# HanielUlises/GCN-GrabCut

Hardware: AMD Instinct MI355X
Metric: images/sec end-to-end mask (DUTS-shape batch) (higher is better)
Workload: dtype f32

## Files before the change

### gcn-grabcut_amd/csrc/ggc_gc.h

```cpp
#pragma once
#include "ggc_internal.h"

namespace ggc {

constexpr int DINF = 1 << 29;

struct GcDims { int B, H, W, P, n_chunks; };

__device__ __forceinline__ int dir_dx(int dir) { return (dir == 0 || dir == 4 || dir == 7) ? -1 : ((dir == 1 || dir == 5 || dir == 6) ? 1 : 0); }
__device__ __forceinline__ int dir_dy(int dir) { return (dir == 2 || dir == 4 || dir == 6) ? -1 : ((dir == 3 || dir == 5 || dir == 7) ? 1 : 0); }
__device__ __forceinline__ int dir_nb(const GcDims& d, int y, int x, int dir) {
    const int yy = y + dir_dy(dir), xx = x + dir_dx(dir);
    if (xx < 0 || xx >= d.W || yy < 0 || yy >= d.H) return -1;
    return yy * d.W + xx;
}

__host__ __device__ __forceinline__ size_t rc_idx(int dir, size_t i) { return i * 8 + (size_t)dir; }

__device__ __forceinline__ void mf_cold_pixel(size_t i, int32_t tw, const int32_t (&cap)[8], int32_t* __restrict__ rc,
                                              int32_t* __restrict__ ex, int32_t* __restrict__ snk, uint8_t* __restrict__ rmask) {
    int arcs = 0;
    int4* r = reinterpret_cast<int4*>(rc + rc_idx(0, i));
    r[0] = make_int4(cap[0], cap[1], cap[2], cap[3]);
    r[1] = make_int4(cap[4], cap[5], cap[6], cap[7]);
#pragma unroll
    for (int dir = 0; dir < 8; ++dir) arcs |= cap[dir] > 0 ? 1 << dir : 0;
    rmask[i] = (uint8_t)arcs;
    ex[i] = tw > 0 ? tw : 0;
    snk[i] = tw < 0 ? -tw : 0;
}

__device__ __forceinline__ void mf_plane_caps(const GcDims& d, int b, int p, const int32_t* __restrict__ nw, int32_t (&cap)[8]) {
    const size_t BP = (size_t)d.B * d.P;
    const int y = p / d.W, x = p % d.W;
    const int32_t* nwb = nw + (size_t)b * d.P;
    const int dirs[4] = {0, 4, 2, 6};
#pragma unroll
    for (int k = 0; k < 4; ++k) {
        const int dir = dirs[k];
        cap[dir] = dir_nb(d, y, x, dir) >= 0 ? nwb[(size_t)k * BP + p] : 0;
        const int q = dir_nb(d, y, x, dir ^ 1);
        cap[dir ^ 1] = q >= 0 ? nwb[(size_t)k * BP + q] : 0;
    }
}

__device__ __forceinline__ void mf_warm_pixel(size_t i, int32_t tw, int32_t tw_old, int32_t* __restrict__ ex,
                                              int32_t* __restrict__ snk) {
    const int32_t bal = (ex[i] - snk[i]) + (tw - tw_old);
    ex[i] = bal > 0 ? bal : 0;
    snk[i] = bal < 0 ? -bal : 0;
}

struct MfControl {
    int32_t* active;
    int32_t* cnt;
    int32_t* lists;
    int32_t* err;
};

int maxflow(ggc_ctx* ctx, hipStream_t st, const GcDims& d, const int32_t* state, int32_t* rc, int32_t* ex,
            int32_t* snk, int32_t* dist, uint8_t* rmask, const MfControl& ctl, bool masks_exact, int& n_open);

constexpr int MF_RT = 32;
constexpr int MF_PT_W = 32, MF_PT_H = 8;
struct MfTiles { int rt_x, rt_y, pt_x, pt_y; };

void mf_zero3(hipStream_t st, int32_t* a, size_t na, int32_t* b, size_t nb, int32_t* c, size_t nc);

constexpr int AQ_HEAD = 0, AQ_TAIL = 32, AQ_PENDING = 64, AQ_DONE = 96, AQ_BUDGET = 97, AQ_VISITS = 128, AQ_WORDS = 160;
int maxflow_relax_async(ggc_ctx* ctx, hipStream_t st, const GcDims& d, const MfTiles& tl, uint8_t* rmask, int32_t* dirty, const int32_t* rc, int32_t* dist,
                        const int32_t* count, const int32_t* list, int32_t* flag, unsigned long long* ring, int32_t* q, int cap,
                        int grid, int32_t* err_flag);
int maxflow_push_async(ggc_ctx* ctx, hipStream_t st, const GcDims& d, const MfTiles& tl, int th, int inner, int gen_max, int32_t* rc,
                       int32_t* ex, int32_t* snk, int32_t* dist, uint8_t* rmask, int32_t* dirty, const int32_t* count, const int32_t* list, int n_list_max, int32_t* state,
                       unsigned long long* ring, int32_t* q, int waves, int32_t* err_flag, long long* prof = nullptr);

}
```

### gcn-grabcut_amd/csrc/ggc_maxflow.hip

```cpp
#include "ggc_gc.h"
#include "ggc_mf_sweep.h"
#include <algorithm>
#include <chrono>
#include <cstdlib>
#include <vector>

namespace ggc {

constexpr int RT = MF_RT;
constexpr int PT_W = MF_PT_W, PT_H = MF_PT_H;
constexpr int PT_N = PT_W * PT_H;
constexpr int PUSH_GRID = 1024, RELAX_GRID = 1024, ASYNC_GRID = 128;

__global__ void __launch_bounds__(256) k_mf_zero3(int32_t* __restrict__ a, size_t na, int32_t* __restrict__ b, size_t nb, int32_t* __restrict__ c, size_t nc) {
    const size_t i = (size_t)blockIdx.x * 256 + threadIdx.x;
    if (i < na) a[i] = 0;
    else if (i < na + nb) b[i - na] = 0;
    else if (i < na + nb + nc) c[i - na - nb] = 0;
}
void mf_zero3(hipStream_t st, int32_t* a, size_t na, int32_t* b, size_t nb, int32_t* c, size_t nc) {
    const size_t n = na + nb + nc;
    if (n) hipLaunchKernelGGL(k_mf_zero3, dim3(cdiv(n, 256)), dim3(256), 0, st, a, na, b, nb, c, nc);
}

// ... 1 lines not shown
struct OutList { int n, base; int buf[OUT_CAP]; };
__device__ __forceinline__ void push_tile_l(int tile, int32_t* __restrict__ flag, OutList& L, int32_t* __restrict__ list,
                                            int32_t* __restrict__ count) {
    if (ldg(&flag[tile]) == 0 && atomicExch(&flag[tile], 1) == 0) {
        const int i = atomicAdd(&L.n, 1);
        if (i < OUT_CAP) L.buf[i] = tile;
        else list[atomicAdd(count, 1)] = tile;
    }
}
__device__ __forceinline__ void flush_tiles(OutList& L, int32_t* __restrict__ list, int32_t* __restrict__ count) {
    __syncthreads();
    const int n = min(L.n, OUT_CAP);
    if (threadIdx.x == 0 && n > 0) L.base = atomicAdd(count, n);
    __syncthreads();
    for (int i = threadIdx.x; i < n; i += blockDim.x) list[L.base + i] = L.buf[i];
}

__global__ void __launch_bounds__(256) k_mf_rinit(GcDims d, MfTiles tl, const int32_t* __restrict__ open_list,
                                                  const int32_t* __restrict__ snk, int32_t* __restrict__ dist,
                                                  int32_t* __restrict__ list, int32_t* __restrict__ flag, int32_t* __restrict__ flag2,
                                                  int32_t* __restrict__ count, int32_t* __restrict__ active, int32_t* __restrict__ scan) {
    constexpr int T = MF_RT;
    __shared__ OutList outl;
    if (threadIdx.x == 0) outl.n = 0;
    if (blockIdx.x == 0 && threadIdx.x == 0) active[open_list[blockIdx.y]] = 0;
    if (blockIdx.x == 0 && blockIdx.y == 0 && threadIdx.x < 8 && (threadIdx.x == 0 || threadIdx.x >= 4)) scan[threadIdx.x] = 0;
    __syncthreads();
    const int tiles_per_image = tl.rt_x * tl.rt_y;
    const int tr = blockIdx.x * 4 + (threadIdx.x >> 6), lane = threadIdx.x & 63;
    if (tr < tiles_per_image) {
        const int b = open_list[blockIdx.y];
        const int ty0 = (tr / tl.rt_x) * T, tx0 = (tr % tl.rt_x) * T;
        const int lx = lane & 31, h = lane >> 5;
        const size_t base = (size_t)b * d.P;
        int sv[16];
#pragma unroll
        for (int r = 0; r < 16; ++r) sv[r] = snk[base + (size_t)min(ty0 + 16 * h + r, d.H - 1) * d.W + min(tx0 + lx, d.W - 1)];
        bool open_px = false;
#pragma unroll
        for (int r = 0; r < 16; ++r) {
            const int y = ty0 + 16 * h + r, x = tx0 + lx;
            if (x < d.W && y < d.H) {
                dist[base + (size_t)y * d.W + x] = sv[r] > 0 ? 1 : DINF;
                open_px |= sv[r] <= 0;
            }
        }
        const bool listed = __any(open_px);
        if (lane == 0) {
            const int tile = b * tiles_per_image + tr;
            flag[tile] = listed ? 1 : 0;
            flag2[tile] = 0;
            if (listed) {
                const int i = atomicAdd(&outl.n, 1);
                if (i < OUT_CAP) outl.buf[i] = tile; else list[atomicAdd(count, 1)] = tile;
            }
        }
    }
    flush_tiles(outl, list, count);
}

template <bool PROF>
__global__ void __launch_bounds__(256) k_mf_relax_wave(GcDims d, MfTiles tl, int phase, long long* __restrict__ prof, uint8_t* __restrict__ rmask,
                                                       int32_t* __restrict__ dirty, const int32_t* __restrict__ rc, int32_t* __restrict__ dist, int32_t* __restrict__ counters,
                                                       const int32_t* __restrict__ list_in, int32_t* __restrict__ list_out,
                                                       int32_t* __restrict__ flag_in, int32_t* __restrict__ flag_out) {
    __shared__ RelaxWaveLds lds[4];
    __shared__ OutList outl;
    if (threadIdx.x == 0) outl.n = 0;
    __syncthreads();
    const int wv = threadIdx.x >> 6;
    const int n_in = counters[phase % 3];
    int32_t* n_out = counters + (phase + 1) % 3;
    if (blockIdx.x == 0 && threadIdx.x == 0) counters[(phase + 2) % 3] = 0;
    const int tiles_per_image = tl.rt_x * tl.rt_y;
    const int G = gridDim.x * 4;
    MfRelaxClocks<PROF> ck;
    int tile_nx = blockIdx.x * 4 + wv < n_in ? list_in[blockIdx.x * 4 + wv] : 0;
    for (int t = blockIdx.x * 4 + wv; t < n_in; t += G) {
        int lane = threadIdx.x & 63;
        asm volatile("" : "+v"(lane));
        ck.begin();
        const int tile = __builtin_amdgcn_readfirstlane(tile_nx);
        tile_nx = t + G < n_in ? list_in[t + G] : 0;
        const int nbm = mf_relax_visit<false, PROF, GGC_MF_RELAX_BFS != 0>(d, tl, tile, lane, lds[wv], rmask, dirty, rc, dist, flag_in, ck);
        const int b = tile / tiles_per_image, tr = tile % tiles_per_image;
        const int tyi = tr / tl.rt_x, txi = tr % tl.rt_x;
        if (lane < 9 && (nbm >> lane) & 1) {
            const int ty = tyi + lane / 3 - 1, tx = txi + lane % 3 - 1;
            if (ty >= 0 && ty < tl.rt_y && tx >= 0 && tx < tl.rt_x)
                push_tile_l(b * tiles_per_image + ty * tl.rt_x + tx, flag_out, outl, list_out, n_out);
        }
        mf_wave_sync();
        ck.end();
    }
    if (PROF && (threadIdx.x & 63) == 0 && ck.sum[3]) {
        unsigned long long* q = reinterpret_cast<unsigned long long*>(prof) + (64 + (blockIdx.x & 63)) * 8;
        for (int k = 0; k < 7; ++k) atomicAdd(&q[k], (unsigned long long)ck.sum[k]);
    }
    flush_tiles(outl, list_out, n_out);
}

__global__ void __launch_bounds__(PT_N) k_mf_pr_list(GcDims d, MfTiles tl, int phase, int inner,
                                                    int32_t* __restrict__ rc, int32_t* __restrict__ ex,
                                                    int32_t* __restrict__ snk, int32_t* __restrict__ dist, uint8_t* __restrict__ rmask,
                                                    int32_t* __restrict__ dirty, int32_t* __restrict__ counters, const int32_t* __restrict__ list_in,
                                                    int32_t* __restrict__ list_out, int32_t* __restrict__ flag_in,
                                                    int32_t* __restrict__ flag_out) {
    __shared__ int s_ex[PT_N];
    __shared__ int s_d[PT_H + 2][PT_W + 2];
    __shared__ int s_rc[8][PT_N];
    __shared__ OutList outl;
    __shared__ int s_nbm;
    const int tid = threadIdx.x, lx = tid & 31;
    if (tid == 0) outl.n = 0;
    const int n_in = counters[phase % 3];
    int32_t* n_out = counters + (phase + 1) % 3;
    if (blockIdx.x == 0 && tid == 0) counters[(phase + 2) % 3] = 0;
    const int tiles_per_image = tl.pt_x * tl.pt_y;
    const size_t BP = (size_t)d.B * d.P;
    constexpr int N_HALO = (PT_H + 2) * (PT_W + 2), HALO_IT = (N_HALO + PT_N - 1) / PT_N;
    struct TileRegs { int e, sk, r[8], hv[HALO_IT]; };
    auto load_tile = [&](int tile, TileRegs& R) {
        const int b = tile / tiles_per_image, tr = tile % tiles_per_image;
        const int tyi = tr / tl.pt_x, txi = tr % tl.pt_x;
        const int x = txi * PT_W + lx;
        const size_t base = (size_t)b * d.P;
        const int y = tyi * PT_H + (tid >> 5);
        const bool in = x < d.W && y < d.H;
        const int p = y * d.W + x;
        R.e = in ? ex[base + p] : 0;
        R.sk = in ? snk[base + p] : 0;
#pragma unroll
        for (int dir = 0; dir < 8; ++dir) R.r[dir] = in ? rc[rc_idx(dir, base + p)] : 0;
#pragma unroll
        for (int k = 0; k < HALO_IT; ++k) {
            const int i = tid + k * PT_N;
            const int gy = tyi * PT_H + i / (PT_W + 2) - 1, gx = txi * PT_W + i % (PT_W + 2) - 1;
            R.hv[k] = (i < N_HALO && gx >= 0 && gx < d.W && gy >= 0 && gy < d.H) ? dist[base + (size_t)gy * d.W + gx] : DINF;
        }
    };
    const int G = gridDim.x;
    int t = blockIdx.x;
    if (t >= n_in) return;
    int tile_next = list_in[t];
    int tile_next2 = t + G < n_in ? list_in[t + G] : 0;
    TileRegs N;
    load_tile(tile_next, N);
    for (; t < n_in; t += G) {
        const int tile = tile_next;
        const int b = tile / tiles_per_image, tr = tile % tiles_per_image;
        const int tyi = tr / tl.pt_x, txi = tr % tl.pt_x;
        const int x = txi * PT_W + lx;
        const size_t base = (size_t)b * d.P;
        __syncthreads();
        const int y = tyi * PT_H + (tid >> 5);
        const bool inb = x < d.W && y < d.H;
        const int pp = y * d.W + x;
        const int e0 = N.e, sk0 = N.sk;
        int sk = sk0, r0[8];
        s_ex[tid] = e0;
#pragma unroll
        for (int dir = 0; dir < 8; ++dir) { r0[dir] = N.r[dir]; s_rc[dir][tid] = r0[dir]; }
#pragma unroll
        for (int k = 0; k < HALO_IT; ++k) {
            const int i = tid + k * PT_N;
            if (i < N_HALO) s_d[i / (PT_W + 2)][i % (PT_W + 2)] = N.hv[k];
        }
        if (t + G < n_in) {
            tile_next = tile_next2;
// ... 203 lines not shown
        launches = phase;
        if (partial) return GGC_OK;
        const int pool = (int)std::min<size_t>(ASYNC_GRID * scale, std::max<size_t>(16, cdiv((size_t)n_cur * per_image, 16)));
        launches = phase + 1;
        return maxflow_relax_async(ctx, st, d, tl, rmask, w.dirty, rc, dist, rl_cnt + phase % 3, w.rl_list[phase & 1], w.rl_flag[phase & 1],
                                   w.ring, w.aq, (int)n_rt, pool, ctl.err);
    }

    int push(int round, int n_cur, size_t scale, int total_active, int& waves) {
        const Knobs& kn = knobs();
        ProfScope ps(ctx, st, "maxflow_push");
        if (round > 0 && total_active <= kn.mf_async_push_active) {
            waves = (int)std::min<long long>(4ll * ASYNC_GRID * (long long)scale, std::max<long long>(64, total_active / 4));
            return maxflow_push_async(ctx, st, d, tl, kn.mf_async_tile, kn.mf_async_sweeps, kn.mf_async_hops, rc, ex, snk, dist, rmask, w.dirty,
                                      pr_cnt, w.pt_list[0], (int)n_pt, w.busy, w.ring, w.aq, waves, ctl.err, prof);
        }
        waves = 0;
        const int launches = round == 0 ? kn.mf_dense_launches0 : kn.mf_dense_launches;
        const int pr_grid = (int)std::min<size_t>(PUSH_GRID * scale, std::max<size_t>(64, (size_t)n_cur * tl.pt_x * tl.pt_y / 2));
        const int grid = (int)std::min<long long>(pr_grid, std::max<long long>(128, 2ll * total_active));
        for (int phase = 0; phase < launches; ++phase)
            hipLaunchKernelGGL(k_mf_pr_list, dim3(grid), dim3(PT_N), 0, st, d, tl, phase, kn.mf_dense_sweeps, rc, ex, snk, dist, rmask, w.dirty, pr_cnt,
                               w.pt_list[phase & 1], w.pt_list[(phase + 1) & 1], w.pt_flag[phase & 1], w.pt_flag[(phase + 1) & 1]);
        GGC_LAUNCH_CHECK(ctx);
        return GGC_OK;
    }
};

struct MfTrace {
    std::chrono::steady_clock::time_point t_prev = std::chrono::steady_clock::now();
    double push_ms = 0.0;

    int round(const MfSolve& s, int round, int n_next, int total_active, int relax_launches) {
        ggc_ctx* ctx = s.ctx;
        long long hh[64 * 8], h[7] = {0, 0, 0, 0, 0, 0, 0};
        GGC_HIP(ctx, hipStreamSynchronize(s.st));
        GGC_HIP(ctx, hipMemcpy(hh, s.prof + 64 * 8, sizeof hh, hipMemcpyDeviceToHost));
        GGC_HIP(ctx, hipMemsetAsync(s.prof + 64 * 8, 0, sizeof hh, s.st));
        for (int i = 0; i < 64; ++i) for (int k = 0; k < 7; ++k) h[k] += hh[i * 8 + k];
        if (h[3] > 0)
            std::fprintf(stderr, "    [relabel visits] %lld dense visits: per visit load+fill %.2f us, sweeps %.2f us (%.1f sweeps, %.1f BFS levels, %lld visits fell back), write-back %.2f us\n",
                         h[3], 0.01 * h[0] / h[3], 0.01 * h[1] / h[3], (double)h[4] / h[3], (double)h[5] / h[3], h[6], 0.01 * h[2] / h[3]);
        std::vector<int32_t> act;
        if (int rcode = read_i32(ctx, s.st, s.ctl.active, s.d.B, act)) return rcode;
        const auto t_now = std::chrono::steady_clock::now();
        const double ms = std::chrono::duration<double, std::milli>(t_now - t_prev).count();
        std::fprintf(stderr, "[ggc maxflow] round %d: open images %d, active pixels %d, relabel launches %d, relabel+scan %.3f ms, previous push %.3f ms\n",
                     round, n_next, total_active, relax_launches, ms - push_ms, push_ms);
        t_prev = t_now;
        if (n_next > 0 && n_next <= 12) {
            std::fprintf(stderr, "    [open]");
            for (int b = 0; b < s.d.B; ++b) if (act[b]) std::fprintf(stderr, " %d:%d", b, act[b]);
            std::fprintf(stderr, "\n");
        }
        return GGC_OK;
    }

    int push(const MfSolve& s, int waves) {
        ggc_ctx* ctx = s.ctx;
        GGC_HIP(ctx, hipStreamSynchronize(s.st));
        push_ms = std::chrono::duration<double, std::milli>(std::chrono::steady_clock::now() - t_prev).count();
        if (waves == 0) return GGC_OK;
        long long hh[128 * 8], h[7] = {0, 0, 0, 0, 0, 0, 0}, g[3] = {0, 0, 0};
        GGC_HIP(ctx, hipMemcpy(hh, s.prof, sizeof hh, hipMemcpyDeviceToHost));
        GGC_HIP(ctx, hipMemsetAsync(s.prof, 0, sizeof hh, s.st));
        for (int i = 0; i < 64; ++i) for (int k = 0; k < 7; ++k) h[k] += hh[i * 8 + k];
        for (int i = 0; i < 64; ++i) for (int k = 0; k < 3; ++k) g[k] += hh[(64 + i) * 8 + k];
        if (h[3] > 0)
            std::fprintf(stderr, "    [async visit] load+fill %.2f us, sweeps %.2f us (%.1f sweeps), write-back+drain %.2f us\n", 0.01 * g[0] / h[3],
                         0.01 * g[1] / h[3], (double)g[2] / h[3], 0.01 * (h[1] - g[0] - g[1]) / h[3]);
        if (h[6] > 0)
            std::fprintf(stderr, "    [async push] %d waves alive %.1f us on average; %lld visits (%lld followed): per visit wait+lock %.2f us, "
                         "visit %.2f us, hand-over %.2f us\n", waves, 0.01 * h[5] / h[6], h[3], h[4], h[3] ? 0.01 * h[0] / h[3] : 0.0,
                         h[3] ? 0.01 * h[1] / h[3] : 0.0, h[3] ? 0.01 * h[2] / h[3] : 0.0);
        return GGC_OK;
    }
};

}

int maxflow(ggc_ctx* ctx, hipStream_t st, const GcDims& d, const int32_t* state, int32_t* rc, int32_t* ex,
            int32_t* snk, int32_t* dist, uint8_t* rmask, const MfControl& ctl, bool masks_exact, int& n_open) {
    const Knobs& kn = knobs();
    const MfTiles tl{cdiv(d.W, RT), cdiv(d.H, RT), cdiv(d.W, PT_W), cdiv(d.H, PT_H)};
    MfSolve s{ctx, st, d, tl, (size_t)tl.rt_x * tl.rt_y * d.B, (size_t)tl.pt_x * tl.pt_y * d.B, rc, ex, snk, dist, rmask,
              ctl, ctl.cnt, ctl.cnt + 1, ctl.cnt + 4, {}, nullptr};
    GGC_REQUIRE(ctx, std::max(s.n_rt, s.n_pt) < (1u << 24), GGC_E_UNSUPPORTED, "batch has more max-flow tiles than a queue entry addresses");
    if (!carve_scratch(ctx, S_GC_M, [&](Carve& c) { s.w.layout(c, s.n_rt, s.n_pt); })) return GGC_E_OOM;
    if (masks_exact) GGC_HIP(ctx, hipMemsetAsync(s.w.dirty, 0, sizeof(int32_t) * s.n_pt, st));
    if (kn.mf_trace) {
        s.prof = s.w.prof;
        GGC_HIP(ctx, hipMemsetAsync(s.prof, 0, 2 * 64 * 8 * sizeof(long long), st));
    }
    GGC_HIP(ctx, hipMemsetAsync(s.n_open, 0, sizeof(int32_t), st));
    int32_t *list_cur = ctl.lists, *list_nxt = ctl.lists + d.B;
    hipLaunchKernelGGL(k_open_init, dim3(cdiv(d.B, 256)), dim3(256), 0, st, d.B, state, list_cur, s.n_open, s.rl_cnt);
    GGC_LAUNCH_CHECK(ctx);
    std::vector<int32_t> host;
    int rcode = GGC_OK;
    if (n_open < 0) {
        if ((rcode = read_i32(ctx, st, s.n_open, 1, host))) return rcode;
        n_open = host[0];
    }
    int n_cur = n_open;
    if (n_cur == 0) return GGC_OK;
    MfTrace trace;
    const int max_rounds = 4096;
    for (int round = 0; round < max_rounds; ++round) {
        const size_t scale = std::max<size_t>(1, ((size_t)n_cur + 32) / 64);
        const bool partial = round < kn.mf_partial_rounds;
        int relax_launches = 0;
        if ((rcode = s.relabel(list_cur, n_cur, scale, partial, relax_launches))) return rcode;
        hipLaunchKernelGGL(k_mf_active, dim3(std::min(cdiv(tl.pt_x * tl.pt_y, 4), 128), n_cur), dim3(256), 0, st, d, tl, list_cur, ex, dist,
                           ctl.active, s.w.pt_flag[0], s.w.pt_flag[1], s.w.pt_list[0], s.pr_cnt);
        hipLaunchKernelGGL(k_done_update, dim3(cdiv(n_cur, 256)), dim3(256), 0, st, n_cur, list_cur, ctl.active, list_nxt, s.n_open, partial ? 1 : 0, s.rl_cnt);
        GGC_LAUNCH_CHECK(ctx);
        if ((rcode = read_i32(ctx, st, s.n_open, 8, host))) return rcode;
        const int n_next = host[0], total_active = host[7];
        if (kn.mf_trace && (rcode = trace.round(s, round, n_next, total_active, relax_launches))) return rcode;
        if (n_next == 0) return GGC_OK;
        std::swap(list_cur, list_nxt);
        int waves = 0;
        if ((rcode = s.push(round, n_cur, scale, total_active, waves))) return rcode;
        if (kn.mf_trace && (rcode = trace.push(s, waves))) return rcode;
        n_cur = n_next;
    }
    return set_err(ctx, GGC_E_DEVICE, "max-flow did not converge in %d rounds", max_rounds);
}

}
```

### gcn-grabcut_amd/csrc/ggc_maxflow_async.hip

```cpp
#include "ggc_gc.h"
#include "ggc_mf_sweep.h"
#include <algorithm>
#include <cstdlib>

namespace ggc {
namespace {

constexpr int PT_H = MF_PT_H;
constexpr long long AQ_TIMEOUT = 200000000ll;

__device__ __forceinline__ unsigned long long ldg64(const unsigned long long* p) { return __hip_atomic_load(p, __ATOMIC_RELAXED, __HIP_MEMORY_SCOPE_AGENT); }
__device__ __forceinline__ void drain() { asm volatile("s_waitcnt vmcnt(0)" ::: "memory"); }

__device__ __forceinline__ int aq_pop(unsigned long long* __restrict__ ring, int32_t* __restrict__ q, int cap, int lane,
                                      int32_t* __restrict__ err_flag) {
    int payload = -1;
    if (lane == 0) {
        const unsigned t = (unsigned)atomicAdd(&q[AQ_HEAD], 1);
        unsigned long long* slot = ring + t % (unsigned)cap;
        const long long t0 = wall_clock64();
        for (int n = 0;; ++n) {
            const unsigned long long v = ldg64(slot);
            if ((unsigned)(v >> 32) == t + 1u) { atomicExch(slot, 0ull); payload = (int)(unsigned)v; break; }
            if ((n & 3) == 3) {
                if (ldg(&q[AQ_DONE]) || ldg(&q[AQ_PENDING]) == 0) break;
                if (wall_clock64() - t0 > AQ_TIMEOUT) { if (err_flag) atomicOr(err_flag, 4); atomicExch(&q[AQ_DONE], 1); break; }
            }
            __builtin_amdgcn_s_sleep(4);
        }
    }
    return __builtin_amdgcn_readfirstlane(payload);
}
__device__ __forceinline__ void aq_push(unsigned long long* __restrict__ ring, int32_t* __restrict__ q, int cap, int payload,
                                        int32_t* __restrict__ err_flag) {
    atomicAdd(&q[AQ_PENDING], 1);
    const unsigned t = (unsigned)atomicAdd(&q[AQ_TAIL], 1);
    unsigned long long* slot = ring + t % (unsigned)cap;
    const unsigned long long e = ((unsigned long long)(t + 1u) << 32) | (unsigned)payload;
    const long long t0 = wall_clock64();
    while (atomicCAS(slot, 0ull, e) != 0ull) {
        if (wall_clock64() - t0 > AQ_TIMEOUT) { if (err_flag) atomicOr(err_flag, 4); atomicExch(&q[AQ_DONE], 1); break; }
        __builtin_amdgcn_s_sleep(2);
    }
}
__device__ __forceinline__ void aq_finish(int32_t* __restrict__ q) {
    if (atomicSub(&q[AQ_PENDING], 1) == 1) atomicExch(&q[AQ_DONE], 1);
}

__global__ void __launch_bounds__(256) k_aq_init(const int32_t* __restrict__ count, const int32_t* __restrict__ list,
                                                 unsigned long long* __restrict__ ring, int32_t* __restrict__ q, int cap, int budget_per_item) {
    const int i = blockIdx.x * blockDim.x + threadIdx.x;
    const int n = min(*count, cap);
    if (i < cap) ring[i] = i < n ? (((unsigned long long)(unsigned)(i + 1)) << 32) | (unsigned)list[i] : 0ull;
    if (i == 0) {
        q[AQ_HEAD] = 0; q[AQ_TAIL] = n; q[AQ_PENDING] = n; q[AQ_DONE] = n == 0 ? 1 : 0; q[AQ_VISITS] = 0;
        q[AQ_BUDGET] = (int)min((long long)n * budget_per_item + 4096, (long long)0x3fffffff);
    }
}

__global__ void __launch_bounds__(256) k_mf_relax_async(GcDims d, MfTiles tl, uint8_t* __restrict__ rmask, int32_t* __restrict__ dirty,
                                                        const int32_t* __restrict__ rc, int32_t* __restrict__ dist, int32_t* __restrict__ flag,
                                                        unsigned long long* __restrict__ ring, int32_t* __restrict__ q, int cap,
                                                        int32_t* __restrict__ err_flag) {
    __shared__ RelaxWaveLds lds[4];
    RelaxWaveLds& S = lds[threadIdx.x >> 6];
    const int tiles_per_image = tl.rt_x * tl.rt_y;
    MfRelaxClocks<false> ck;
    int tile = -1;
    for (;;) {
        int lane = threadIdx.x & 63;
        asm volatile("" : "+v"(lane));
        if (tile < 0) {
            tile = aq_pop(ring, q, cap, lane, err_flag);
            if (tile < 0) break;
            if (lane == 0) atomicExch(&flag[tile], 0);
            drain();
        }
        const int nbm = mf_relax_visit<true, false>(d, tl, tile, lane, S, rmask, dirty, rc, dist, flag, ck);
        drain();
        const int b = tile / tiles_per_image, tr = tile % tiles_per_image;
        const int tyi = tr / tl.rt_x, txi = tr % tl.rt_x;
        int nb = -1;
        if (lane < 9 && (nbm >> lane) & 1) {
            const int ty = tyi + lane / 3 - 1, tx = txi + lane % 3 - 1;
            if (ty >= 0 && ty < tl.rt_y && tx >= 0 && tx < tl.rt_x) nb = b * tiles_per_image + ty * tl.rt_x + tx;
        }
        const bool cand = nb >= 0 && ldg(&flag[nb]) == 0;
        const unsigned long long cm = __ballot(cand);
        int next = -1;
        if (cm) {
            const int fl = __ffsll((long long)cm) - 1;
            next = __shfl(nb, fl, 64);
            if (cand && lane != fl && atomicExch(&flag[nb], 1) == 0) aq_push(ring, q, cap, nb, err_flag);
            drain();
        }
        if (next < 0 && lane == 0) aq_finish(q);
        tile = next;
        mf_wave_sync();
    }
}

constexpr int ST_Q = 1, ST_BUSY = 2;

template <int TH>
struct PushTileLds {
    int ex[32 * TH]; int sk[32 * TH]; int d[TH + 2][34]; int rc[8][32 * TH];
    uint32_t mask[32]; unsigned short list[32 * TH];
};

template <int TH>
__device__ int push_tile_visit(const GcDims& d, int tyi, int txi, int inner, size_t base, size_t BP,
                               int32_t* __restrict__ rc, int32_t* __restrict__ ex, int32_t* __restrict__ snk,
                               int32_t* __restrict__ dist, uint8_t* __restrict__ rmask, PushTileLds<TH>& S, int lane,
                               bool prof, long long (&pv)[4]) {
    constexpr int NPX = TH / 2, HALO = (TH + 2) * 34, HALO_IT = (HALO + 63) / 64;
    const long long tv0 = prof ? wall_clock64() : 0;
    const int lx = lane & 31, r0 = lane >> 5;
    const int x = txi * 32 + lx;
    int e0[NPX], sk0[NPX], r0v[NPX][8];
#pragma unroll
    for (int j = 0; j < NPX; ++j) {
        const int y = tyi * TH + r0 + 2 * j;
        const int pc = min(y, d.H - 1) * d.W + min(x, d.W - 1);
        e0[j] = ldg(ex + base + pc);
        sk0[j] = ldg(snk + base + pc);
#pragma unroll
        for (int dir = 0; dir < 8; ++dir) r0v[j][dir] = ldg(rc + rc_idx(dir, base + pc));
    }
    int* sd = &S.d[0][0];
    int hv[HALO_IT];
#pragma unroll
    for (int k = 0; k < HALO_IT; ++k) {
        const int i = min(lane + k * 64, HALO - 1);
        const int gy = tyi * TH + i / 34 - 1, gx = txi * 32 + i % 34 - 1;
        hv[k] = ldg(dist + base + (size_t)min(max(gy, 0), d.H - 1) * d.W + min(max(gx, 0), d.W - 1));
    }
#pragma unroll
    for (int k = 0; k < HALO_IT; ++k) {
        const int i = lane + k * 64;
        const int gy = tyi * TH + i / 34 - 1, gx = txi * 32 + i % 34 - 1;
        if (i < HALO) sd[i] = (gx >= 0 && gx < d.W && gy >= 0 && gy < d.H) ? hv[k] : DINF;
    }
    if (lane < 32) S.mask[lane] = 0u;
    mf_wave_sync();
#pragma unroll
    for (int j = 0; j < NPX; ++j) {
        const int slot = lane + 64 * j, ly = r0 + 2 * j;
        const bool inb = x < d.W && tyi * TH + ly < d.H;
        if (!inb) { e0[j] = 0; sk0[j] = 0; }
        S.ex[slot] = e0[j];
        S.sk[slot] = sk0[j];
#pragma unroll
        for (int dir = 0; dir < 8; ++dir) {
            if (!inb) r0v[j][dir] = 0;
            S.rc[dir][slot] = r0v[j][dir];
        }
        const bool a = e0[j] > 0 && S.d[ly + 1][lx + 1] < d.P;
        const unsigned long long m = __ballot(a);
        if (lane == 0) { S.mask[2 * j] = (uint32_t)m; S.mask[2 * j + 1] = (uint32_t)(m >> 32); }
    }
    mf_wave_sync();
    int nbm = 0;
    const long long tv1 = prof ? wall_clock64() : 0;
    int n_sw = 0;
// ... 248 lines not shown
```

### gcn-grabcut_amd/csrc/ggc_mf_sweep.h

```cpp
#pragma once
#include "ggc_gc.h"

namespace ggc {

__device__ __forceinline__ void mf_wave_sync() {
    __builtin_amdgcn_fence(__ATOMIC_ACQ_REL, "wavefront");
    __builtin_amdgcn_wave_barrier();
}
__device__ __forceinline__ int ldg(const int32_t* p) { return __hip_atomic_load(p, __ATOMIC_RELAXED, __HIP_MEMORY_SCOPE_AGENT); }
__device__ __forceinline__ int mf_wave_or(int v) {
#pragma unroll
    for (int o = 32; o > 0; o >>= 1) v |= __shfl_xor(v, o, 64);
    return v;
}

struct RelaxWaveLds { int d[MF_RT + 2][MF_RT + 2]; uint32_t m[MF_RT][MF_RT / 4]; };

__device__ __forceinline__ int gated(int v, uint32_t inv, int bit) {
    return (__builtin_amdgcn_sbfe((int)inv, bit, 1) & DINF) | v;
}
__device__ __forceinline__ int min3i(int a, int b, int c) { return min(a, min(b, c)); }
template <int bA, int bB, int bC, int bD, int bE>
__device__ __forceinline__ int relax_px5(int c, uint32_t inv, int pos, int vA, int vB, int vC, int vD, int vE) {
    const int nd = min3i(min3i(gated(vA, inv, pos + bA), gated(vB, inv, pos + bB), gated(vC, inv, pos + bC)),
                         gated(vD, inv, pos + bD), gated(vE, inv, pos + bE));
    return min(c, nd + 1);
}


struct MfBorderArcs {
    int fr[4][3], fc[3];
    __device__ __forceinline__ void load(const GcDims& d, const int32_t* __restrict__ rc, size_t BP, size_t base, int ty0, int tx0,
                                         int lx, int h) {
        const size_t cx = min(tx0 + lx, d.W - 1);
#pragma unroll
        for (int q = 0; q < 4; ++q) {
            const int r = (q >> 1) * 8 + ((q & 1) ? 7 : 0);
            const size_t i = base + (size_t)min(ty0 + 16 * h + r, d.H - 1) * d.W + cx;
#pragma unroll
            for (int t = 0; t < 3; ++t) fr[q][t] = rc[rc_idx(((q & 1) ? 3 + 2 * t : 2 + 2 * t), i)];
        }
        const size_t i = base + (size_t)min(ty0 + lx, d.H - 1) * d.W + min(tx0 + (h ? 31 : 0), d.W - 1);
        fc[0] = rc[rc_idx((h ? 1 : 0), i)];
        fc[1] = rc[rc_idx((h ? 5 : 4), i)];
        fc[2] = rc[rc_idx((h ? 6 : 7), i)];
    }
    __device__ __forceinline__ uint32_t row(uint32_t m, int r) const {
        if ((r & 7) == 0 || (r & 7) == 7) {
            const int q = (r >> 3) * 2 + ((r & 7) ? 1 : 0);
#pragma unroll
            for (int t = 0; t < 3; ++t) {
                const uint32_t bit = 1u << (((r & 7) ? 3 : 2) + 2 * t);
                m = (fr[q][t] > 0) ? (m & ~bit) : (m | bit);
            }
        }
        return m;
    }
    __device__ __forceinline__ uint32_t col(uint32_t m, int h) const {
        const uint32_t b0 = 1u << (h ? 1 : 0), b1 = 1u << (h ? 5 : 4), b2 = 1u << (h ? 6 : 7);
        m = (fc[0] > 0) ? (m & ~b0) : (m | b0);
        m = (fc[1] > 0) ? (m & ~b1) : (m | b1);
        m = (fc[2] > 0) ? (m & ~b2) : (m | b2);
        return m;
    }
};

__device__ __forceinline__ bool mf_tile_dirty(const int32_t* __restrict__ dirty, const MfTiles& tl, int b, int tyi, int txi, int lane) {
    const int py = tyi * (MF_RT / MF_PT_H) + (lane & 3);
    const int v = (lane < 4 && py < tl.pt_y) ? dirty[(size_t)b * tl.pt_x * tl.pt_y + (size_t)py * tl.pt_x + txi] : 0;
    return __any(v != 0);
}
__device__ __forceinline__ void mf_tile_repair(const GcDims& d, const MfTiles& tl, uint8_t* __restrict__ rmask, int32_t* __restrict__ dirty,
                                               const RelaxWaveLds& S, size_t base, int b, int tyi, int txi, int ty0, int tx0, int lx, int h, int lane) {
    const uint8_t* sm = reinterpret_cast<const uint8_t*>(&S.m[0][0]);
#pragma unroll
    for (int q = 0; q < 4; ++q) {
        const int r = (q >> 1) * 8 + ((q & 1) ? 7 : 0);
        const int y = ty0 + 16 * h + r, x = tx0 + lx;
        if (x < d.W && y < d.H) rmask[base + (size_t)y * d.W + x] = (uint8_t)(~sm[(16 * h + r) * MF_RT + lx] & 0xffu);
    }
    {
        const int y = ty0 + lx, x = tx0 + (h ? 31 : 0);
        if (x < d.W && y < d.H) rmask[base + (size_t)y * d.W + x] = (uint8_t)(~sm[lx * MF_RT + (h ? 31 : 0)] & 0xffu);
    }
    const int py = tyi * (MF_RT / MF_PT_H) + (lane & 3);
    if (lane < 4 && py < tl.pt_y) dirty[(size_t)b * tl.pt_x * tl.pt_y + (size_t)py * tl.pt_x + txi] = 0;
}

__device__ __forceinline__ int relax_sweep_v(RelaxWaveLds& S, const uint32_t (&inv_in)[4], int lx, int h) {
    uint32_t inv[4] = {inv_in[0], inv_in[1], inv_in[2], inv_in[3]};
    asm volatile("" : "+v"(inv[0]), "+v"(inv[1]), "+v"(inv[2]), "+v"(inv[3]));
    int w[18][3];
#pragma unroll
    for (int a = 0; a < 18; ++a)
#pragma unroll
        for (int c = 0; c < 3; ++c) w[a][c] = S.d[16 * h + a][lx + c];
    uint32_t chg = 0;
#pragma unroll
    for (int r = 0; r < 16; ++r) {
// ... 89 lines not shown
    uint32_t A[8] = {0u, 0u, 0u, 0u, 0u, 0u, 0u, 0u};
#pragma unroll
    for (int g = 0; g < 4; ++g) {
        const uint64_t x = bit_transpose8((uint64_t)S.m[r][2 * g] | (uint64_t)S.m[r][2 * g + 1] << 32);
#pragma unroll
        for (int dir = 0; dir < 8; ++dir) A[dir] |= (uint32_t)((x >> (8 * dir)) & 0xffu) << (8 * g);
    }
#pragma unroll
    for (int dir = 0; dir < 8; ++dir) A[dir] = ~A[dir];
    const int eL = mf_entry3(S.d[r][0], ~A[4], S.d[r + 1][0], ~A[0], S.d[r + 2][0], ~A[7]);
    const int eR = mf_entry3(S.d[r][T + 1], ~A[6] >> 31, S.d[r + 1][T + 1], ~A[1] >> 31, S.d[r + 2][T + 1], ~A[5] >> 31);
    const uint32_t ib = sm[(h ? T - 1 : 0) * T + r];
    const int hr = h ? T + 1 : 0;
    const int eTB = mf_entry3(S.d[hr][r], ib >> (h ? 7 : 4), S.d[hr][r + 1], ib >> (h ? 3 : 2), S.d[hr][r + 2], ib >> (h ? 5 : 6));
    uint32_t one = 0u;
#pragma unroll
    for (int q = 0; q < 16; ++q) {
        const unsigned long long bal = __ballot(old[q] == 1);
        one = (r == q) ? (uint32_t)bal : one;
        one = (r == 16 + q) ? (uint32_t)(bal >> 32) : one;
    }
    mf_wave_sync();
    uint32_t done = 0u, front = 0u, pl[7] = {0u, 0u, 0u, 0u, 0u, 0u, 0u};
    const int up_lane = (r == 0 ? lane : lane - 1) * 4, dn_lane = (r == T - 1 ? lane : lane + 1) * 4;
    const uint32_t up_ok = r == 0 ? 0u : ~0u, dn_ok = r == T - 1 ? 0u : ~0u;
    auto next_level = [&]() {
        int c = (one & ~done) ? 1 : DINF;
        c = min(c, (done & 1u) ? DINF : eL);
        c = min(c, (done >> 31) ? DINF : eR);
        const uint32_t d0 = __builtin_amdgcn_readlane(done, 0), d31 = __builtin_amdgcn_readlane(done, 31);
        c = min(c, (((h ? d31 : d0) >> r) & 1u) ? DINF : eTB);
        return __builtin_amdgcn_readfirstlane(mf_wave_min(c));
    };
    int L = next_level();
    bool finished = L >= DINF;
    for (int k = 0; k < MF_BFS_CAP && !finished; ++k) {
        if (lane == 0) lv[k] = L;
        const unsigned long long tb = __ballot(eTB == L);
        uint32_t own = (eL == L ? 1u : 0u) | (eR == L ? 0x80000000u : 0u);
        own |= ((uint32_t)tb & ~up_ok) | ((uint32_t)(tb >> 32) & ~dn_ok);
        if (L == 1) own |= one;
        const uint32_t fu = (uint32_t)__builtin_amdgcn_ds_bpermute(up_lane, (int)front) & up_ok;
        const uint32_t fd = (uint32_t)__builtin_amdgcn_ds_bpermute(dn_lane, (int)front) & dn_ok;
        const uint32_t reach = (A[0] & (front << 1)) | (A[1] & (front >> 1)) | (A[2] & fu) | (A[3] & fd) |
                               (A[4] & (fu << 1)) | (A[5] & (fd >> 1)) | (A[6] & (fu >> 1)) | (A[7] & (fd << 1));
        const uint32_t nw = (reach | own) & ~done;
        done |= nw;
#pragma unroll
        for (int j = 0; j < 7; ++j) pl[j] |= ((k >> j) & 1) ? nw : 0u;
        front = nw;
        if (PROF) ++ck.n_lv;
        if (__any(nw != 0u)) ++L;
        else { L = next_level(); finished = L >= DINF; }
    }
    if (!finished) return false;
    mf_wave_sync();
    uint32_t viol = 0u;
#pragma unroll
    for (int g = 0; g < 2; ++g) {
        uint64_t x = 0;
#pragma unroll
        for (int j = 0; j < 7; ++j) x |= (uint64_t)((pl[j] >> (16 * h + 8 * g)) & 0xffu) << (8 * j);
        x = bit_transpose8(x);
#pragma unroll
        for (int i = 0; i < 8; ++i) {
            const int c = 16 * h + 8 * g + i;
            const bool reached = (done >> c) & 1u;
            const int start = S.d[r + 1][c + 1];
            const int b = reached ? lv[(int)((x >> (8 * i)) & 0x7fu)] : DINF;
            viol |= reached ? (uint32_t)(start < b) : (uint32_t)(start != DINF);
            if (b < start) S.d[r + 1][c + 1] = b;
        }
    }
    mf_wave_sync();
    if (__any(viol != 0u)) {
#pragma unroll
        for (int q = 0; q < 16; ++q) S.d[16 * h + q + 1][r + 1] = old[q];
        mf_wave_sync();
        return false;
    }
    return true;
}

template <bool ASYNC, bool PROF, bool BFS = false>
__device__ __forceinline__ int mf_relax_visit(const GcDims& d, const MfTiles& tl, int tile, int lane, RelaxWaveLds& S,
                                              uint8_t* rmask, int32_t* dirty, const int32_t* rc,
                                              int32_t* dist, int32_t* flag, MfRelaxClocks<PROF>& ck) {
    constexpr int T = MF_RT, N_HALO = (T + 2) * (T + 2), HALO_IT = (N_HALO + 63) / 64;
    int* sd = &S.d[0][0];
    uint8_t* sm = reinterpret_cast<uint8_t*>(&S.m[0][0]);
    const int tiles_per_image = tl.rt_x * tl.rt_y;
    const int b = tile / tiles_per_image, tr = tile % tiles_per_image;
    const int tyi = tr / tl.rt_x, txi = tr % tl.rt_x;
    const int tx0 = txi * T, ty0 = tyi * T;
    const size_t base = (size_t)b * d.P, BP = (size_t)d.B * d.P;
    const int lx = lane & 31, h = lane >> 5;
    int hv[HALO_IT];
#pragma unroll
    for (int k = 0; k < HALO_IT; ++k) {
        const int i = min(lane + k * 64, N_HALO - 1);
        const int gy = ty0 + i / (T + 2) - 1, gx = tx0 + i % (T + 2) - 1;
        const int32_t* p = &dist[base + (size_t)min(max(gy, 0), d.H - 1) * d.W + min(max(gx, 0), d.W - 1)];
        hv[k] = ASYNC ? ldg(p) : *p;
    }
    uint32_t mv[16];
#pragma unroll
    for (int r = 0; r < 16; ++r)
        mv[r] = rmask[base + (size_t)min(ty0 + 16 * h + r, d.H - 1) * d.W + min(tx0 + lx, d.W - 1)];
    const bool dirty_t = mf_tile_dirty(dirty, tl, b, tyi, txi, lane);
    MfBorderArcs ba;
    if (dirty_t) ba.load(d, rc, BP, base, ty0, tx0, lx, h);
    if (!ASYNC && lane == 0) flag[tile] = 0;
    uint32_t inv_v[4] = {0u, 0u, 0u, 0u}, inv_h[4];
#pragma unroll
    for (int r = 0; r < 16; ++r) {
        uint32_t m = ~mv[r] & 0xffu;
        if (dirty_t) m = ba.row(m, r);
        sm[(16 * h + r) * T + lx] = (uint8_t)((tx0 + lx < d.W && ty0 + 16 * h + r < d.H) ? m : 0xffu);
    }
#pragma unroll
    for (int k = 0; k < HALO_IT; ++k) {
        const int i = lane + k * 64;
        const int gy = ty0 + i / (T + 2) - 1, gx = tx0 + i % (T + 2) - 1;
        if (i < N_HALO) sd[i] = (gx >= 0 && gx < d.W && gy >= 0 && gy < d.H) ? hv[k] : DINF;
    }
    mf_wave_sync();
    if (dirty_t) {
        if (ty0 + lx < d.H && tx0 + (h ? 31 : 0) < d.W) sm[lx * T + (h ? 31 : 0)] = (uint8_t)ba.col(sm[lx * T + (h ? 31 : 0)], h);
        mf_wave_sync();
        mf_tile_repair(d, tl, rmask, dirty, S, base, b, tyi, txi, ty0, tx0, lx, h, lane);
    }
#pragma unroll
    for (int r = 0; r < 16; ++r) inv_v[r >> 2] |= (uint32_t)sm[(16 * h + r) * T + lx] << (8 * (r & 3));
#pragma unroll
    for (int k = 0; k < 4; ++k) inv_h[k] = S.m[lx][4 * h + k];
    int old[16];
#pragma unroll
    for (int r = 0; r < 16; ++r) old[r] = S.d[16 * h + r + 1][lx + 1];
    bool settled = false;
    ck.t1 = ck.now();
    if (BFS) {
        settled = mf_relax_visit_bfs<PROF>(S, old, lane, ck);
        if (PROF && !settled) ck.n_fb = 1;
    }
    for (int it = 0; it < 4 * T && !(BFS && settled); ++it) {
        const int ch = (it & 1) ? relax_sweep_h(S, inv_h, lx, h) : relax_sweep_v(S, inv_v, lx, h);
        mf_wave_sync();
        if (PROF) ++ck.n_sw;
        if (!__any(ch)) { settled = true; break; }
    }
    ck.t2 = ck.now();
    int nbm = settled ? 0 : 1 << 4;
#pragma unroll
    for (int r = 0; r < 16; ++r) {
        const int ly = 16 * h + r;
        const int v = S.d[ly + 1][lx + 1];
        if (v != old[r]) {
            int32_t* p = &dist[base + (size_t)(ty0 + ly) * d.W + tx0 + lx];
            if (ASYNC) atomicMin(p, v); else *p = v;
            const int Lf = lx == 0, Rt = lx == T - 1, U = ly == 0, D = ly == T - 1;
            nbm |= (U & Lf) | U << 1 | (U & Rt) << 2 | Lf << 3 | Rt << 5 | (D & Lf) << 6 | D << 7 | (D & Rt) << 8;
        }
    }
    return mf_wave_or(nbm);
}

}
```

Before: 3842.

## Restructure relax-visit tile loads: interior rows, ring halo, vectorized mask reads

The relax tile visit now loads the 32x32 interior labels directly into registers, one column per lane, and fetches the halo ring separately. Previously it gathered the whole 34x34 halo with per-element div/mod index math. The residual mask is read as one 16-byte load per lane when the width and pointer alignment allow, with a byte fallback otherwise. Tile-index div/mod is replaced by precomputed reciprocal multiplication, and the old values come from registers instead of being re-read from LDS. The changes aim to cut integer address arithmetic and memory instructions in a hot, frequently launched kernel. In exchange the code adds alignment preconditions and a more intricate border-arc handling path.

```diff
diff --git a/gcn-grabcut_amd/csrc/ggc_gc.h b/gcn-grabcut_amd/csrc/ggc_gc.h
--- a/gcn-grabcut_amd/csrc/ggc_gc.h
+++ b/gcn-grabcut_amd/csrc/ggc_gc.h
@@ -63,7 +63,22 @@
 
 constexpr int MF_RT = 32;
 constexpr int MF_PT_W = 32, MF_PT_H = 8;
-struct MfTiles { int rt_x, rt_y, pt_x, pt_y; };
+struct MfTiles { int rt_x, rt_y, pt_x, pt_y; uint32_t rcp_rt_x, rcp_per_image; };
+
+__host__ __device__ __forceinline__ uint32_t mf_rcp(uint32_t dv) { return dv > 1u ? (uint32_t)((1ull << 32) / dv) : 0xffffffffu; }
+__host__ __device__ __forceinline__ uint32_t mf_divmod(uint32_t n, uint32_t dv, uint32_t rcp, uint32_t& rem) {
+    uint32_t q = (uint32_t)(((uint64_t)n * rcp) >> 32);
+    rem = n - q * dv;
+    if (rem >= dv) { ++q; rem -= dv; }
+    return q;
+}
+struct MfTilePos { int b, tyi, txi; };
+__host__ __device__ __forceinline__ MfTilePos mf_tile_pos(const MfTiles& tl, int tile) {
+    uint32_t tr, txi;
+    const uint32_t b = mf_divmod((uint32_t)tile, (uint32_t)(tl.rt_x * tl.rt_y), tl.rcp_per_image, tr);
+    const uint32_t tyi = mf_divmod(tr, (uint32_t)tl.rt_x, tl.rcp_rt_x, txi);
+    return {(int)b, (int)tyi, (int)txi};
+}
 
 void mf_zero3(hipStream_t st, int32_t* a, size_t na, int32_t* b, size_t nb, int32_t* c, size_t nc);
 
diff --git a/gcn-grabcut_amd/csrc/ggc_maxflow.hip b/gcn-grabcut_amd/csrc/ggc_maxflow.hip
--- a/gcn-grabcut_amd/csrc/ggc_maxflow.hip
+++ b/gcn-grabcut_amd/csrc/ggc_maxflow.hip
@@ -107,9 +107,9 @@
         ck.begin();
         const int tile = __builtin_amdgcn_readfirstlane(tile_nx);
         tile_nx = t + G < n_in ? list_in[t + G] : 0;
-        const int nbm = mf_relax_visit<false, PROF, GGC_MF_RELAX_BFS != 0>(d, tl, tile, lane, lds[wv], rmask, dirty, rc, dist, flag_in, ck);
-        const int b = tile / tiles_per_image, tr = tile % tiles_per_image;
-        const int tyi = tr / tl.rt_x, txi = tr % tl.rt_x;
+        const MfTilePos at = mf_tile_pos(tl, tile);
+        const int nbm = mf_relax_visit<false, PROF, GGC_MF_RELAX_BFS != 0>(d, tl, tile, at, lane, lds[wv], rmask, dirty, rc, dist, flag_in, ck);
+        const int b = at.b, tyi = at.tyi, txi = at.txi;
         if (lane < 9 && (nbm >> lane) & 1) {
             const int ty = tyi + lane / 3 - 1, tx = txi + lane % 3 - 1;
             if (ty >= 0 && ty < tl.rt_y && tx >= 0 && tx < tl.rt_x)
@@ -479,7 +479,8 @@
 int maxflow(ggc_ctx* ctx, hipStream_t st, const GcDims& d, const int32_t* state, int32_t* rc, int32_t* ex,
             int32_t* snk, int32_t* dist, uint8_t* rmask, const MfControl& ctl, bool masks_exact, int& n_open) {
     const Knobs& kn = knobs();
-    const MfTiles tl{cdiv(d.W, RT), cdiv(d.H, RT), cdiv(d.W, PT_W), cdiv(d.H, PT_H)};
+    const MfTiles tl{cdiv(d.W, RT), cdiv(d.H, RT), cdiv(d.W, PT_W), cdiv(d.H, PT_H),
+                     mf_rcp((uint32_t)cdiv(d.W, RT)), mf_rcp((uint32_t)(cdiv(d.W, RT) * cdiv(d.H, RT)))};
     MfSolve s{ctx, st, d, tl, (size_t)tl.rt_x * tl.rt_y * d.B, (size_t)tl.pt_x * tl.pt_y * d.B, rc, ex, snk, dist, rmask,
               ctl, ctl.cnt, ctl.cnt + 1, ctl.cnt + 4, {}, nullptr};
     GGC_REQUIRE(ctx, std::max(s.n_rt, s.n_pt) < (1u << 24), GGC_E_UNSUPPORTED, "batch has more max-flow tiles than a queue entry addresses");
diff --git a/gcn-grabcut_amd/csrc/ggc_maxflow_async.hip b/gcn-grabcut_amd/csrc/ggc_maxflow_async.hip
--- a/gcn-grabcut_amd/csrc/ggc_maxflow_async.hip
+++ b/gcn-grabcut_amd/csrc/ggc_maxflow_async.hip
@@ -76,10 +76,11 @@
             if (lane == 0) atomicExch(&flag[tile], 0);
             drain();
         }
-        const int nbm = mf_relax_visit<true, false>(d, tl, tile, lane, S, rmask, dirty, rc, dist, flag, ck);
+        tile = __builtin_amdgcn_readfirstlane(tile);
+        const MfTilePos at = mf_tile_pos(tl, tile);
+        const int nbm = mf_relax_visit<true, false>(d, tl, tile, at, lane, S, rmask, dirty, rc, dist, flag, ck);
         drain();
-        const int b = tile / tiles_per_image, tr = tile % tiles_per_image;
-        const int tyi = tr / tl.rt_x, txi = tr % tl.rt_x;
+        const int b = at.b, tyi = at.tyi, txi = at.txi;
         int nb = -1;
         if (lane < 9 && (nbm >> lane) & 1) {
             const int ty = tyi + lane / 3 - 1, tx = txi + lane % 3 - 1;
diff --git a/gcn-grabcut_amd/csrc/ggc_mf_sweep.h b/gcn-grabcut_amd/csrc/ggc_mf_sweep.h
--- a/gcn-grabcut_amd/csrc/ggc_mf_sweep.h
+++ b/gcn-grabcut_amd/csrc/ggc_mf_sweep.h
@@ -14,7 +14,8 @@
     return v;
 }
 
-struct RelaxWaveLds { int d[MF_RT + 2][MF_RT + 2]; uint32_t m[MF_RT][MF_RT / 4]; };
+struct alignas(16) RelaxWaveLds { int d[MF_RT + 2][MF_RT + 2]; uint32_t m[MF_RT][MF_RT / 4]; };
+static_assert(sizeof(RelaxWaveLds) % 16 == 0 && (sizeof(int) * (MF_RT + 2) * (MF_RT + 2)) % 16 == 0, "m and its half rows are 16-byte aligned: the visit stores them as uint4");
 
 __device__ __forceinline__ int gated(int v, uint32_t inv, int bit) {
     return (__builtin_amdgcn_sbfe((int)inv, bit, 1) & DINF) | v;
@@ -270,61 +271,117 @@
     return true;
 }
 
+struct MfLd { uint32_t off; bool in; };
+struct MfCell { int wy, wx; };
+__host__ __device__ __forceinline__ int mf_clampi(int v, int lo, int hi) { return v < lo ? lo : (v > hi ? hi : v); }
+__host__ __device__ __forceinline__ uint32_t mf_ld_row(int H, int W, int gy) { return (uint32_t)mf_clampi(gy, 0, H - 1) * (uint32_t)W; }
+
+__host__ __device__ __forceinline__ MfCell mf_interior_cell(int lane, int r) { return {16 * (lane >> 5) + r + 1, (lane & 31) + 1}; }
+__host__ __device__ __forceinline__ int mf_interior_rows(int H, int W, int ty0, int tx0, int lane) {
+    return tx0 + (lane & 31) < W ? mf_clampi(H - ty0 - 16 * (lane >> 5), 0, 16) : 0;
+}
+__host__ __device__ __forceinline__ uint32_t mf_interior_step(int W, int nv, int r) { return r < nv ? (uint32_t)W : 0u; }
+__host__ __device__ __forceinline__ uint32_t mf_ld_interior(int H, int W, int ty0, int tx0, int lane, int r) {
+    uint32_t off = mf_ld_row(H, W, ty0 + 16 * (lane >> 5)) + (uint32_t)mf_clampi(tx0 + (lane & 31), 0, W - 1);
+    const int nv = mf_interior_rows(H, W, ty0, tx0, lane);
+    for (int k = 1; k <= r; ++k) off += mf_interior_step(W, nv, k);
+    return off;
+}
+__host__ __device__ __forceinline__ bool mf_ring_stores(int lane, int k) { return k == 2 || lane < MF_RT + 2; }
+__host__ __device__ __forceinline__ MfCell mf_ring_cell(int lane, int k) {
+    if (k == 2) return {(lane & 31) + 1, (lane >> 5) ? MF_RT + 1 : 0};
+    return {k ? MF_RT + 1 : 0, lane < MF_RT + 1 ? lane : MF_RT + 1};
+}
+__host__ __device__ __forceinline__ MfLd mf_ld_ring(int H, int W, int ty0, int tx0, int lane, int k) {
+    const MfCell c = mf_ring_cell(lane, k);
+    const int gy = ty0 + c.wy - 1, gx = tx0 + c.wx - 1;
+    return {mf_ld_row(H, W, gy) + (uint32_t)mf_clampi(gx, 0, W - 1), gy >= 0 && gy < H && gx >= 0 && gx < W};
+}
+__host__ __device__ __forceinline__ bool mf_mask16_ok(int W, const void* rmask) { return ((uint32_t)W & 15u) == 0u && ((uintptr_t)rmask & 15u) == 0u; }
+__host__ __device__ __forceinline__ MfLd mf_ld_mask16(int H, int W, int ty0, int tx0, int lane) {
+    const int gy = ty0 + (lane >> 1), gx = tx0 + 16 * (lane & 1);
+    return {mf_ld_row(H, W, gy) + (uint32_t)mf_clampi(gx, 0, W - 16), gy < H && gx < W};
+}
+
+template <bool ASYNC>
+__device__ __forceinline__ int mf_load_label(const int32_t* p) { return ASYNC ? ldg(p) : *p; }
+
 template <bool ASYNC, bool PROF, bool BFS = false>
-__device__ __forceinline__ int mf_relax_visit(const GcDims& d, const MfTiles& tl, int tile, int lane, RelaxWaveLds& S,
+__device__ __forceinline__ int mf_relax_visit(const GcDims& d, const MfTiles& tl, int tile, const MfTilePos& at, int lane, RelaxWaveLds& S,
                                               uint8_t* rmask, int32_t* dirty, const int32_t* rc,
                                               int32_t* dist, int32_t* flag, MfRelaxClocks<PROF>& ck) {
-    constexpr int T = MF_RT, N_HALO = (T + 2) * (T + 2), HALO_IT = (N_HALO + 63) / 64;
-    int* sd = &S.d[0][0];
+    constexpr int T = MF_RT;
     uint8_t* sm = reinterpret_cast<uint8_t*>(&S.m[0][0]);
-    const int tiles_per_image = tl.rt_x * tl.rt_y;
-    const int b = tile / tiles_per_image, tr = tile % tiles_per_image;
-    const int tyi = tr / tl.rt_x, txi = tr % tl.rt_x;
+    const int b = at.b, tyi = at.tyi, txi = at.txi;
     const int tx0 = txi * T, ty0 = tyi * T;
     const size_t base = (size_t)b * d.P, BP = (size_t)d.B * d.P;
     const int lx = lane & 31, h = lane >> 5;
-    int hv[HALO_IT];
-#pragma unroll
-    for (int k = 0; k < HALO_IT; ++k) {
-        const int i = min(lane + k * 64, N_HALO - 1);
-        const int gy = ty0 + i / (T + 2) - 1, gx = tx0 + i % (T + 2) - 1;
-        const int32_t* p = &dist[base + (size_t)min(max(gy, 0), d.H - 1) * d.W + min(max(gx, 0), d.W - 1)];
-        hv[k] = ASYNC ? ldg(p) : *p;
-    }
+    const int32_t* db = dist + base;
+    const int nv = mf_interior_rows(d.H, d.W, ty0, tx0, lane);
+    int old[16], rv[3];
+    {
+        const int32_t* p = db + mf_ld_interior(d.H, d.W, ty0, tx0, lane, 0);
+#pragma unroll
+        for (int r = 0; r < 16; ++r) {
+            if (r) p += mf_interior_step(d.W, nv, r);
+            old[r] = mf_load_label<ASYNC>(p);
+        }
+    }
+#pragma unroll
+    for (int k = 0; k < 3; ++k) rv[k] = mf_load_label<ASYNC>(db + mf_ld_ring(d.H, d.W, ty0, tx0, lane, k).off);
+    const bool wide = mf_mask16_ok(d.W, rmask);
+    const MfLd m16 = mf_ld_mask16(d.H, d.W, ty0, tx0, lane);
+    uint4 mq = make_uint4(0u, 0u, 0u, 0u);
     uint32_t mv[16];
-#pragma unroll
-    for (int r = 0; r < 16; ++r)
-        mv[r] = rmask[base + (size_t)min(ty0 + 16 * h + r, d.H - 1) * d.W + min(tx0 + lx, d.W - 1)];
+    if (wide) mq = *reinterpret_cast<const uint4*>(rmask + base + m16.off);
+    else {
+        const uint8_t* p = rmask + base + mf_ld_interior(d.H, d.W, ty0, tx0, lane, 0);
+#pragma unroll
+        for (int r = 0; r < 16; ++r) {
+            if (r) p += mf_interior_step(d.W, nv, r);
+            mv[r] = *p;
+        }
+    }
     const bool dirty_t = mf_tile_dirty(dirty, tl, b, tyi, txi, lane);
     MfBorderArcs ba;
     if (dirty_t) ba.load(d, rc, BP, base, ty0, tx0, lx, h);
     if (!ASYNC && lane == 0) flag[tile] = 0;
-    uint32_t inv_v[4] = {0u, 0u, 0u, 0u}, inv_h[4];
+    int* sdl = &S.d[16 * h + 1][lx + 1];
 #pragma unroll
     for (int r = 0; r < 16; ++r) {
-        uint32_t m = ~mv[r] & 0xffu;
-        if (dirty_t) m = ba.row(m, r);
-        sm[(16 * h + r) * T + lx] = (uint8_t)((tx0 + lx < d.W && ty0 + 16 * h + r < d.H) ? m : 0xffu);
-    }
-#pragma unroll
-    for (int k = 0; k < HALO_IT; ++k) {
-        const int i = lane + k * 64;
-        const int gy = ty0 + i / (T + 2) - 1, gx = tx0 + i % (T + 2) - 1;
-        if (i < N_HALO) sd[i] = (gx >= 0 && gx < d.W && gy >= 0 && gy < d.H) ? hv[k] : DINF;
+        old[r] = r < nv ? old[r] : DINF;
+        sdl[r * (T + 2)] = old[r];
+    }
+#pragma unroll
+    for (int k = 0; k < 3; ++k) {
+        const MfCell c = mf_ring_cell(lane, k);
+        const int v = mf_ld_ring(d.H, d.W, ty0, tx0, lane, k).in ? rv[k] : DINF;
+        if (mf_ring_stores(lane, k)) S.d[c.wy][c.wx] = v;
+    }
+    if (wide) {
+        const uint4 v = m16.in ? make_uint4(~mq.x, ~mq.y, ~mq.z, ~mq.w) : make_uint4(~0u, ~0u, ~0u, ~0u);
+        *reinterpret_cast<uint4*>(&S.m[lane >> 1][4 * (lane & 1)]) = v;
+    } else {
+#pragma unroll
+        for (int r = 0; r < 16; ++r) sm[(16 * h + r) * T + lx] = (uint8_t)(r < nv ? ~mv[r] & 0xffu : 0xffu);
     }
     mf_wave_sync();
     if (dirty_t) {
+#pragma unroll
+        for (int q = 0; q < 4; ++q) {
+            const int r = (q >> 1) * 8 + ((q & 1) ? 7 : 0);
+            if (r < nv) sm[(16 * h + r) * T + lx] = (uint8_t)ba.row(sm[(16 * h + r) * T + lx], r);
+        }
+        mf_wave_sync();
         if (ty0 + lx < d.H && tx0 + (h ? 31 : 0) < d.W) sm[lx * T + (h ? 31 : 0)] = (uint8_t)ba.col(sm[lx * T + (h ? 31 : 0)], h);
         mf_wave_sync();
         mf_tile_repair(d, tl, rmask, dirty, S, base, b, tyi, txi, ty0, tx0, lx, h, lane);
     }
+    uint32_t inv_v[4] = {0u, 0u, 0u, 0u}, inv_h[4];
 #pragma unroll
     for (int r = 0; r < 16; ++r) inv_v[r >> 2] |= (uint32_t)sm[(16 * h + r) * T + lx] << (8 * (r & 3));
 #pragma unroll
     for (int k = 0; k < 4; ++k) inv_h[k] = S.m[lx][4 * h + k];
-    int old[16];
-#pragma unroll
-    for (int r = 0; r < 16; ++r) old[r] = S.d[16 * h + r + 1][lx + 1];
     bool settled = false;
     ck.t1 = ck.now();
     if (BFS) {
```

Measured after the change: 3820. About the same (-0.6%).
